# PolyChord/PolyChordLite

Measured on AMD Instinct MI355X. Metric: likelihood evals/sec, 20D Gaussian nlive=2000, higher is better.
Workload: dtype f64; 1 GPU; configs[1]: 20-D Gaussian, nlive=2000, num_repeats=40, one full run per step; batch_chains=1000, parallelism=repeat-sharded x1, mode=one run at a time per GPU; R runs in step: roofline.in_step

## Files before the change

### polychordlite_amd/csrc/pc_sample.hip

```cpp
#include "pc_state.h"
#ifndef __HIPCC_RTC__
#include <cstdlib>
#endif

template <int DPL>
struct LaneDims {
    double lo[DPL], span[DPL];
    double mean[DPL];
    bool on[DPL];
};

__device__ __forceinline__ double pc_box_theta(double lo, double span, double cube) { return lo + span * cube; }
#define PC_PT_SORTED (1u << 16)
#define PC_PT_PERMUTED (1u << 17)
#define PC_PT_ADAPTIVE (1u << 18)
#define PC_PT_LAYER (1u << 19)
template <int DPL>
struct LaneTable {
    int type[DPL], pos[DPL], len[DPL], hyp[DPL];
    int cnt[DPL], lay[DPL];
    double p0[DPL], p1[DPL], p2[DPL];
    unsigned mask;
};
template <int DPL, bool AD>
// ... 1011 lines not shown
    if (off > 0) {
        for (int e = tid; e < Dg * D; e += NT) G[e] = 0.0;
        __syncthreads();
    }
    for (uint32_t call = (e0 >> 1) + tid; call <= ((e1 - 1) >> 1); call += NT) {
        double ua, ub;
        if (S.seq_mode) pc_uniform2(S.k0, S.k1, PC_DOM_SEQ, 0u, 0u, call, ua, ub);
        else pc_uniform2(S.k0, S.k1, PC_DOM_NHAT, batch, (uint32_t)chain, call, ua, ub);
        const uint32_t ia = 2 * call, ib = 2 * call + 1;
        if (ia >= e0 && ia < e1) { const uint32_t x = ia - e0; G[off == 0 ? x : (x / Dg) * D + off + x % Dg] = pc_inv_normal_cdf(ua); }
        if (ib >= e0 && ib < e1) { const uint32_t x = ib - e0; G[off == 0 ? x : (x / Dg) * D + off + x % Dg] = pc_inv_normal_cdf(ub); }
    }
    __syncthreads();
#ifdef NHATS_DBG
    ncyc[2] = clock64();
#endif
#pragma unroll
    for (int d = 0; d < DMAX; ++d) v[d] = (active && d < D) ? G[(size_t)i * D + d] : 0.0;
#define PC_DOT4(RES, A, B) { double p0_ = 0.0, p1_ = 0.0, p2_ = 0.0, p3_ = 0.0; \
        _Pragma("unroll") for (int d = 0; d < DMAX; d += 4) { \
            p0_ += (A)[d] * (B)[d]; p1_ += (A)[d + 1] * (B)[d + 1]; p2_ += (A)[d + 2] * (B)[d + 2]; p3_ += (A)[d + 3] * (B)[d + 3]; } \
        RES = (p0_ + p1_) + (p2_ + p3_); }
    {
        double n2;
        PC_DOT4(n2, v, v)
        const double inrm = 1.0 / sqrt(n2);
#pragma unroll
        for (int d = 0; d < DMAX; ++d) v[d] = v[d] * inrm;
    }
#ifdef NHATS_DBG
    ncyc[3] = clock64();
#endif
    double *Qb = Q;
    const int QS = DMAX;
    if (i == 0) {
#pragma unroll
        for (int d = 0; d < DMAX; ++d) Qb[d] = v[d];
    }
    __syncthreads();
#define PC_GS_STEP(QV) { \
        double qq, dv; \
        PC_DOT4(qq, QV, QV) \
        PC_DOT4(dv, QV, v) \
        if (i == j) { \
            const double inrm = 1.0 / sqrt(qq); \
            _Pragma("unroll") for (int d = 0; d < DMAX; ++d) v[d] = v[d] * inrm; \
        } else if (active && i > j) { \
            const double cproj = dv / qq; \
            _Pragma("unroll") for (int d = 0; d < DMAX; ++d) v[d] = v[d] - cproj * (QV)[d]; \
            if (i == j + 1) { \
                double *qn = Qb + (size_t)((j + 1) & 1) * QS; \
                _Pragma("unroll") for (int d = 0; d < DMAX; ++d) qn[d] = v[d]; \
            } \
        } }
    for (int j = 0; j < Dg; ++j) {
        const double *q = Qb + (size_t)(j & 1) * QS;
        if constexpr (DMAX <= 32) {
            double qv[DMAX];
#pragma unroll
            for (int d = 0; d < DMAX; ++d) qv[d] = q[d];
            PC_GS_STEP(qv)
        } else {
            PC_GS_STEP(q)
        }
        __syncthreads();
    }
#undef PC_GS_STEP
    if constexpr (PART == 1) {
        if (active) {
#pragma unroll
            for (int d = 0; d < DMAX; ++d) if (d < D) raw[d] = v[d];
        }
        return;
    }
    }
#ifdef NHATS_DBG
    ncyc[4] = clock64();
#endif
    const int col = col0 + basis * Dg + i;
    const bool wanted = basis * Dg + i < nrg;
    if constexpr (DMAX <= 32) {
        const double *Lg = S.chol + (size_t)sh[0] * D * D;
        for (int e = tid; e < D * D; e += NT) G[e] = Lg[e];
        __syncthreads();
        if (active && wanted) {
            double t[DMAX];
#pragma unroll
            for (int a = 0; a < DMAX; ++a) t[a] = 0.0;
#pragma unroll
            for (int b = 0; b < DMAX; ++b)
#pragma unroll
                for (int a = b; a < DMAX; ++a) t[a] += G[(size_t)a * D + b] * v[b];
#pragma unroll
            for (int a = 0; a < DMAX; ++a) if (a >= D) t[a] = 0.0;
            double n2;
            PC_DOT4(n2, t, t)
            const double w = sqrt(n2), iw = 1.0 / w;
            double *out = S.nhat + ((size_t)chain * nr + col) * D;
#pragma unroll
            for (int d = 0; d < DMAX; ++d) if (d < D) out[d] = t[d] * iw;
            S.nhat_w[(size_t)chain * nr + col] = w * 3.0;
        }
    } else {
        const int DS = D + 1, TR = 12;
        double *Lt = G + (size_t)D * DS;
        __syncthreads();
        if (active) {
#pragma unroll
            for (int d = 0; d < DMAX; ++d) if (d < D) G[(size_t)i * DS + d] = v[d];
        }
        const double *Lc = S.chol + (size_t)sh[0] * D * D;
        double *mine = G + (size_t)i * DS;
        for (int a_hi = D - 1; a_hi >= 0; a_hi -= TR) {
            const int a_lo = max(0, a_hi - TR + 1), nrow = a_hi - a_lo + 1;
            __syncthreads();
            for (int e = tid; e < nrow * D; e += NT) Lt[e] = Lc[(size_t)a_lo * D + e];
            __syncthreads();
            if (active && wanted) {
                for (int a = a_hi; a >= a_lo; --a) {
                    const double *Lr = Lt + (size_t)(a - a_lo) * D;
                    double t0 = 0.0, t1 = 0.0, t2 = 0.0, t3 = 0.0;
                    int bb = 0;
                    for (; bb + 3 <= a; bb += 4) {
                        t0 += Lr[bb] * mine[bb]; t1 += Lr[bb + 1] * mine[bb + 1]; t2 += Lr[bb + 2] * mine[bb + 2]; t3 += Lr[bb + 3] * mine[bb + 3];
                    }
                    for (; bb <= a; ++bb) t0 += Lr[bb] * mine[bb];
                    mine[a] = (t0 + t1) + (t2 + t3);
                }
            }
        }
        if (active && wanted) {
            double n0 = 0.0, n1 = 0.0;
            int d = 0;
            for (; d + 1 < D; d += 2) { n0 += mine[d] * mine[d]; n1 += mine[d + 1] * mine[d + 1]; }
            if (d < D) n0 += mine[d] * mine[d];
            const double w = sqrt(n0 + n1);
            Q[i] = 1.0 / w;
            S.nhat_w[(size_t)chain * nr + col] = w * 3.0;
        }
        __syncthreads();
        for (int r = 0; r < Dg && basis * Dg + r < nrg; ++r) {
            double *out = S.nhat + ((size_t)chain * nr + col0 + basis * Dg + r) * D;
            const double iw = Q[r];
            for (int d = tid; d < D; d += NT) out[d] = G[(size_t)r * DS + d] * iw;
        }
    }
#ifdef NHATS_DBG
    ncyc[5] = clock64();
    if (tid == 0 && blockIdx.x == 0 && blockIdx.y == 0) for (int x = 0; x < 5; ++x) S.ctl->dbg[x] += ncyc[x + 1] - ncyc[x];
#endif
#undef PC_DOT4
}

template <int DMAX>
__global__ __launch_bounds__(64) void k_nhats_w(PcState S, unsigned batch, int nbases)
{
    extern __shared__ __attribute__((aligned(16))) char smem[];
    const int D = S.D, DD = D * D, nb = S.nb_total, nr = S.nr, per = 64 / D, NC = (DD + 1) / 2;
    const int tid = threadIdx.x, sub = tid / D, i = tid - sub * D;
    const int g0 = blockIdx.x * per, g = g0 + sub;
    const int nbw = nbases - g0 < per ? nbases - g0 : per;
    const bool active = sub < per && g < nbases;
    double *G = (double *)smem;
    double *Qw = G + (size_t)per * DD;
    int *qA = (int *)(Qw + (size_t)per * 2 * DMAX);
    if (nr <= 64) {
        for (int s = 0; s < nbw; ++s) {
            const int chain = (g0 + s) / nb;
            if (g0 + s != chain * nb) continue;
            const int dk = pc_deck_keyed(S, batch, chain, tid, nr);
            int *rec = pc_deck_record(S, chain);
            rec[2 + tid] = dk;
            const unsigned long long tg = pc_deck_tag(S, batch, chain, nr);
            if (tid == 0) { rec[0] = (int)(unsigned)tg; rec[1] = (int)(unsigned)(tg >> 32); }
        }
    }
    int qn = 0;
    auto put = [&](bool want, double u, int dst) {
        bool t = false;
        double x = 0.0;
        if (want) x = pc_inv_normal_central(u, t);
        if (want) G[dst] = t ? u : x;
        const unsigned long long m = __ballot(want && t);
        if (want && t) qA[qn + __popcll(m & ((1ull << tid) - 1ull))] = dst;
        qn += __popcll(m);
    };
    for (int t0 = 0; t0 < nbw * NC; t0 += 64) {
        const int t = t0 + tid;
        const bool in = t < nbw * NC;
        const int s = in ? t / NC : 0, m = in ? t - s * NC : 0;
        const int chain = (g0 + s) / nb, basis = (g0 + s) - chain * nb;
        const uint32_t e0 = (uint32_t)pc_sel(S.g_e0, 0) + (uint32_t)basis * DD, e1 = e0 + (uint32_t)DD;
        const uint32_t call = (e0 >> 1) + (uint32_t)m;
        double ua = 0.5, ub = 0.5;
        if (in) pc_uniform2(S.k0, S.k1, PC_DOM_NHAT, batch, (uint32_t)chain, call, ua, ub);
        const uint32_t ia = 2 * call, ib = ia + 1;
        put(in && ia >= e0 && ia < e1, ua, s * DD + (int)(ia - e0));
        put(in && ib >= e0 && ib < e1, ub, s * DD + (int)(ib - e0));
    }
    __syncthreads();
    for (int k = tid; k < qn; k += 64) { const int at = qA[k]; G[at] = pc_inv_normal_tail(G[at]); }
    __syncthreads();
    double v[DMAX];
    const double *mine = G + (size_t)(active ? sub : 0) * DD + (size_t)i * D;
#pragma unroll
    for (int d = 0; d < DMAX; ++d) v[d] = (active && d < D) ? mine[d] : 0.0;
    double *Q = Qw + (size_t)(sub < per ? sub : 0) * 2 * DMAX;
    {
#pragma clang fp contract(off)
        PC_GS_PACKED(DMAX, v, Q, D, i, active)
    }
    if (active) {
        double *raw = S.nhat_raw + ((size_t)g * D + i) * D;
#pragma unroll
        for (int d = 0; d < DMAX; ++d) if (d < D) raw[d] = v[d];
    }
}

#define PC_BIG_NT 256
#define PC_BIG_P 16
__global__ __launch_bounds__(PC_BIG_NT) void k_nhats_big(PcState S, unsigned batch)
{
    __shared__ int sh[2];
    __shared__ double iwv[PC_BIG_NT];
    __shared__ double Pq[PC_BIG_P * PC_BIG_NT];
    __shared__ double pqq[PC_BIG_P];
    const int D = S.D, nr = S.nr, tid = threadIdx.x, chain = blockIdx.y, i = tid;
    int grade, basis;
    pc_grade_of_basis(S, blockIdx.x, grade, basis);
    const int off = pc_sel(S.g_off, grade), Dg = D - off, nrg = pc_sel(S.g_nr, grade), col0 = pc_sel(S.g_col0, grade);
    if (tid == 0) {
        int sel, slot;
        select_seed(S, batch, chain, sel, slot);
        sh[0] = sel; sh[1] = slot;
        if (blockIdx.x == 0) {
            S.ch_cluster[chain] = sel; S.ch_seed_slot[chain] = slot;
            S.ch_contour[chain] = S.logLp[sel];
            S.ch_epoch[chain] = S.ctl->admin_epoch;
            if (chain == 0) { S.ctl->i_nursery = gridDim.y; S.ctl->batch_id = batch; }
        }
    }
    double *V = S.nhat_raw + ((size_t)chain * gridDim.x + blockIdx.x) * D * PC_BIG_NT;
    const int nvec = min(Dg, nrg - basis * Dg);
    const bool active = i < nvec;
    const uint32_t eoff = S.seq_mode ? (uint32_t)S.ctl->seq + 2u : 0u;
    const uint32_t e0 = eoff + (uint32_t)pc_sel(S.g_e0, grade) + (uint32_t)basis * Dg * Dg, e1 = e0 + (uint32_t)Dg * Dg;
    for (int e = tid; e < off * PC_BIG_NT; e += PC_BIG_NT) V[e] = 0.0;
    for (uint32_t call = (e0 >> 1) + tid; call <= ((e1 - 1) >> 1); call += PC_BIG_NT) {
        double ua, ub;
        if (S.seq_mode) pc_uniform2(S.k0, S.k1, PC_DOM_SEQ, 0u, 0u, call, ua, ub);
        else pc_uniform2(S.k0, S.k1, PC_DOM_NHAT, batch, (uint32_t)chain, call, ua, ub);
        const uint32_t ia = 2 * call, ib = 2 * call + 1;
        if (ia >= e0 && ia < e1) { const uint32_t x = ia - e0; V[(size_t)(off + x % Dg) * PC_BIG_NT + x / Dg] = pc_inv_normal_cdf(ua); }
        if (ib >= e0 && ib < e1) { const uint32_t x = ib - e0; V[(size_t)(off + x % Dg) * PC_BIG_NT + x / Dg] = pc_inv_normal_cdf(ub); }
    }
    __syncthreads();
    double *mine = V + i;
    auto dot_own = [&](const double *q) {
        double p0 = 0.0, p1 = 0.0, p2 = 0.0, p3 = 0.0;
        int d = off;
        for (; d + 3 < D; d += 4) {
            p0 += q[(size_t)d * PC_BIG_NT] * mine[(size_t)d * PC_BIG_NT]; p1 += q[(size_t)(d + 1) * PC_BIG_NT] * mine[(size_t)(d + 1) * PC_BIG_NT];
            p2 += q[(size_t)(d + 2) * PC_BIG_NT] * mine[(size_t)(d + 2) * PC_BIG_NT]; p3 += q[(size_t)(d + 3) * PC_BIG_NT] * mine[(size_t)(d + 3) * PC_BIG_NT];
        }
        for (; d < D; ++d) p0 += q[(size_t)d * PC_BIG_NT] * mine[(size_t)d * PC_BIG_NT];
        return (p0 + p1) + (p2 + p3);
    };
    auto norm2 = [&](const double *q) {
        double p0 = 0.0, p1 = 0.0, p2 = 0.0, p3 = 0.0;
        int d = off;
        for (; d + 3 < D; d += 4) {
            const double a = q[(size_t)d * PC_BIG_NT], b = q[(size_t)(d + 1) * PC_BIG_NT], c = q[(size_t)(d + 2) * PC_BIG_NT], e = q[(size_t)(d + 3) * PC_BIG_NT];
            p0 += a * a; p1 += b * b; p2 += c * c; p3 += e * e;
        }
        for (; d < D; ++d) { const double a = q[(size_t)d * PC_BIG_NT]; p0 += a * a; }
        return (p0 + p1) + (p2 + p3);
    };
    if (active) {
        const double inrm = 1.0 / sqrt(dot_own(mine));
        for (int d = off; d < D; ++d) mine[(size_t)d * PC_BIG_NT] *= inrm;
    }
    __syncthreads();
    {
        const int wv = tid >> 6, lane = tid & 63;
        for (int j0 = 0; j0 < nvec; j0 += PC_BIG_P) {
            const int np = min(PC_BIG_P, nvec - j0);
            for (int e = tid; e < np * D; e += PC_BIG_NT) {
                const int pp = e % np, d = e / np;
                Pq[pp * PC_BIG_NT + d] = V[(size_t)d * PC_BIG_NT + j0 + pp];
            }
            for (int e = np * PC_BIG_NT + tid; e < PC_BIG_P * PC_BIG_NT; e += PC_BIG_NT) Pq[e] = 0.0;
            __syncthreads();
            for (int pp = 0; pp + 1 < np; ++pp) {
                const double *qp = Pq + pp * PC_BIG_NT;
                for (int q = pp + 1 + wv; q < np; q += 4) {
                    double *vq = Pq + q * PC_BIG_NT;
                    double dq = 0.0, dd = 0.0;
                    for (int d = off + lane; d < D; d += 64) { const double a = qp[d], b2 = vq[d]; dq += a * b2; dd += a * a; }
                    dq = wave_sum<4>(dq); dd = wave_sum<4>(dd);
                    const double c = dq / dd;
                    for (int d = off + lane; d < D; d += 64) vq[d] -= c * qp[d];
                }
                __syncthreads();
            }
            for (int pp = wv; pp < np; pp += 4) {
                const double *qp = Pq + pp * PC_BIG_NT;
                double dd = 0.0;
                for (int d = off + lane; d < D; d += 64) dd += qp[d] * qp[d];
                dd = wave_sum<4>(dd);
                if (lane == 0) pqq[pp] = dd;
            }
            for (int e = tid; e < np * D; e += PC_BIG_NT) {
                const int pp = e % np, d = e / np;
                V[(size_t)d * PC_BIG_NT + j0 + pp] = Pq[pp * PC_BIG_NT + d];
            }
            __syncthreads();
            if (active && i >= j0 + np) {
                double c[PC_BIG_P];
#pragma unroll
                for (int pp = 0; pp < PC_BIG_P; ++pp) c[pp] = 0.0;
                for (int d = off; d < D; ++d) {
                    const double x = mine[(size_t)d * PC_BIG_NT];
#pragma unroll
                    for (int pp = 0; pp < PC_BIG_P; ++pp) c[pp] += x * Pq[pp * PC_BIG_NT + d];
                }
#pragma unroll
                for (int pp = 0; pp < PC_BIG_P; ++pp) c[pp] = pp < np ? c[pp] / pqq[pp] : 0.0;
                for (int d = off; d < D; ++d) {
                    double x = mine[(size_t)d * PC_BIG_NT];
#pragma unroll
                    for (int pp = 0; pp < PC_BIG_P; ++pp) x -= c[pp] * Pq[pp * PC_BIG_NT + d];
                    mine[(size_t)d * PC_BIG_NT] = x;
                }
            }
            __syncthreads();
        }
    }
    if (active) {
        const double inrm = 1.0 / sqrt(dot_own(mine));
        for (int d = off; d < D; ++d) mine[(size_t)d * PC_BIG_NT] *= inrm;
    }
    {
        const double *Lc = S.chol + (size_t)sh[0] * D * D;
        for (int a_hi = D - 1; a_hi >= 0; a_hi -= PC_BIG_P) {
            const int a_lo = max(0, a_hi - PC_BIG_P + 1), nrow = a_hi - a_lo + 1;
            __syncthreads();
            for (int e = tid; e < PC_BIG_P * PC_BIG_NT; e += PC_BIG_NT) {
                const int r = e / PC_BIG_NT, b2 = e % PC_BIG_NT;
                Pq[e] = (r < nrow && b2 <= a_hi) ? Lc[(size_t)(a_lo + r) * D + b2] : 0.0;
            }
            __syncthreads();
            if (active) {
                double acc[PC_BIG_P];
#pragma unroll
                for (int r = 0; r < PC_BIG_P; ++r) acc[r] = 0.0;
                for (int b2 = 0; b2 <= a_hi; ++b2) {
                    const double x = mine[(size_t)b2 * PC_BIG_NT];
#pragma unroll
                    for (int r = 0; r < PC_BIG_P; ++r) acc[r] += Pq[r * PC_BIG_NT + b2] * x;
                }
#pragma unroll
                for (int r = 0; r < PC_BIG_P; ++r) if (r < nrow) mine[(size_t)(a_lo + r) * PC_BIG_NT] = acc[r];
            }
        }
    }
    if (active) {
        double sn = 0.0, cn = 0.0;
        for (int d = 0; d < D; ++d) {
#pragma clang fp contract(off)
// ... 550 lines not shown
        if (kind == PC_LIKE_SOURCE) {
            lA = oa ? C.S.logzero : like_eval<DPL, NROWS, KIND>(C.S, thA, C.ld, C.lane, C.ybuf);
            lB = ob ? C.S.logzero : like_eval<DPL, NROWS, KIND>(C.S, thB, C.ld, C.lane, C.ybuf);
            if (!oa && lA > C.S.logzero) C.nlike++;
            if (!ob && lB > C.S.logzero) C.nlike++;
            return;
        }
#endif
        lA = like_eval<DPL, NROWS, KIND>(C.S, thA, C.ld, C.lane, C.ybuf);
        lB = like_eval<DPL, NROWS, KIND>(C.S, thB, C.ld, C.lane, C.ybuf);
        if (oa) lA = C.S.logzero; else if (lA > C.S.logzero) C.nlike++;
        if (ob) lB = C.S.logzero; else if (lB > C.S.logzero) C.nlike++;
        return;
    }
    bool outA = false, outB = false;
    double sA = 0.0, sB = 0.0, s2A = 0.0, s2B = 0.0;
#pragma unroll
    for (int k = 0; k < DPL; ++k) {
        const double cA = x0[k] + tA * nh[k], cB = x0[k] + tB * nh[k];
        if (C.ld.on[k]) { outA |= (cA < 0.0) | (cA > 1.0); outB |= (cB < 0.0) | (cB > 1.0); }
        const double thA = C.ld.lo[k] + C.ld.span[k] * cA, thB = C.ld.lo[k] + C.ld.span[k] * cB;
        if (C.ld.on[k]) {
            if (kind == PC_LIKE_RASTRIGIN) {
                sA += 8.515435146961291 + thA * thA - 10.0 * cos(PC_TWO_PI * thA);
                sB += 8.515435146961291 + thB * thB - 10.0 * cos(PC_TWO_PI * thB);
            } else {
                const int dim = C.lane + 64 * k;
                const double m1 = dim < 2 ? -0.5 : 0.0, m2 = dim < 2 ? 0.5 : 0.0;
                const double a1 = (thA - m1) * L.inv_sigma, a2 = (thA - m2) * L.inv_sigma;
                const double b1 = (thB - m1) * L.inv_sigma, b2 = (thB - m2) * L.inv_sigma;
                sA += a1 * a1; s2A += a2 * a2; sB += b1 * b1; s2B += b2 * b2;
            }
        }
    }
    const bool oa = __ballot(outA) != 0ull, ob = __ballot(outB) != 0ull;
    sA = wsum<DPL, NROWS>(sA); sB = wsum<DPL, NROWS>(sB);
    if (kind == PC_LIKE_RASTRIGIN) { lA = -sA; lB = -sB; }
    else {
        s2A = wsum<DPL, NROWS>(s2A); s2B = wsum<DPL, NROWS>(s2B);
        lA = pc_logaddexp(L.norm - sA / 2.0, L.norm - s2A / 2.0) - 0.6931471805599453;
        lB = pc_logaddexp(L.norm - sB / 2.0, L.norm - s2B / 2.0) - 0.6931471805599453;
    }
    if (oa) lA = C.S.logzero; else if (lA > C.S.logzero) C.nlike++;
    if (ob) lB = C.S.logzero; else if (lB > C.S.logzero) C.nlike++;
}

#ifndef PC_STEP_SPEC
#define PC_STEP_SPEC 1
#endif
constexpr int pc_step_spec = PC_STEP_SPEC;
#ifdef PC_SLICE_WAVES
#define PC_SLICE_ATTR __attribute__((amdgpu_waves_per_eu(PC_SLICE_WAVES, PC_SLICE_WAVES)))
#else
#define PC_SLICE_ATTR
#endif
template <int DPL, int NROWS, bool SPECIAL, int WPB = 1, int FW = 0, int LEAN = 0, int PT = 0>
__global__ PC_SLICE_ATTR __launch_bounds__(64 * WPB * ((FW > 0 && (LEAN == 1 || LEAN == 3 || LEAN == 5) && WPB == 4) ? 2 : 1)) void k_slice(PcState S, unsigned batch, int phi_lds, int mat_lds)
{
#include "pc_slice_body.inc"
}

template <int DPL, int NROWS, bool SPECIAL, int WPB = 1, int FW = 0, int LEAN = 0, int PT = 0>
__global__ PC_SLICE_ATTR __launch_bounds__(64 * WPB) void k_slice_many(const PcManyRec *__restrict__ R, int phi_lds, int mat_lds)
{
    const PcState S = R[blockIdx.y].S;
    const unsigned batch = (unsigned)R[blockIdx.y].ia[PC_REC_I_BATCH];
#include "pc_slice_body.inc"
}

#ifndef __HIPCC_RTC__
#include "pc_launch.h"
#include <cstdio>
extern "C" int pc_rtc_wanted(const PcState *S) { return S->like.kind == PC_LIKE_SOURCE || (S->ablate & PC_ABL_RTC_BUILTINS) != 0; }
template <class... A> static int pc_rtc_go(const PcState *S, const char *expr, dim3 g, dim3 b, size_t sh, hipStream_t st, A... a)
{
    void *args[] = { (void *)&a... };
    return pc_rtc_launch(S, expr, g, b, sh, st, args);
}
#define PC_LAUNCH(K, G, B, SH, ST, ...) do { if (pc_rtc_wanted(S)) { if (pc_rtc_go(S, #K, G, B, SH, ST, __VA_ARGS__)) return 1; } \
                                             else hipLaunchKernelGGL(K, G, B, SH, ST, __VA_ARGS__); } while (0)
static size_t pc_terms_lds(const PcState *S, const PcSourceForm &f, int phi_lds)
{
    if (f.nterms <= 0) return 0;
    return sizeof(double) * ((size_t)S->D + (phi_lds ? (size_t)S->nr * (size_t)f.nsums : 0)) + pc_front_lds(f);
}
static PcSourceForm pc_state_form(const PcState *S)
{
    PcSourceForm f{};
    if (S->like.kind == PC_LIKE_SOURCE) (void)pc_rtc_source_form(S->src_id, &f);
    return f;
}
static int pc_dpl(int D) { return D <= 64 ? 1 : (D <= 128 ? 2 : (D <= 256 ? 4 : 0)); }
extern "C" int pc_launch_generate_live(const PcState *S, int attempt0, int n, double *rows, double *rows_logL,
                                       hipStream_t st)
{
    const size_t sh = sizeof(double) * S->D + pc_front_lds(pc_state_form(S));
    const bool table = S->prior.kind >= 2;
    switch (pc_dpl(S->D) + (table ? 8 : 0)) {
    case 1: PC_LAUNCH((k_generate_live<1>), dim3(n), dim3(64), sh, st, *S, attempt0, rows, rows_logL); return 0;
    case 2: PC_LAUNCH((k_generate_live<2>), dim3(n), dim3(64), sh, st, *S, attempt0, rows, rows_logL); return 0;
    case 4: PC_LAUNCH((k_generate_live<4>), dim3(n), dim3(64), sh, st, *S, attempt0, rows, rows_logL); return 0;
    case 9: PC_LAUNCH((k_generate_live<1, 1>), dim3(n), dim3(64), sh, st, *S, attempt0, rows, rows_logL); return 0;
    case 10: PC_LAUNCH((k_generate_live<2, 1>), dim3(n), dim3(64), sh, st, *S, attempt0, rows, rows_logL); return 0;
    case 12: PC_LAUNCH((k_generate_live<4, 1>), dim3(n), dim3(64), sh, st, *S, attempt0, rows, rows_logL); return 0;
    }
    return 1;
}

extern "C" int pc_nhats_splittable(const PcState *S)
{
    const char *e = std::getenv("PC_NHATS_QUAD_MIN");
    if (S->D > 64 && S->D <= 128) return S->ngrade <= 1 && !S->seq_mode && S->nhat_raw != nullptr;
    if (S->D > 24 && S->D <= 64) return S->ngrade <= 1 && !S->seq_mode && S->nhat_raw != nullptr && (!e || std::atoi(e) <= 25);
    return S->D <= 24 && S->D < (e ? std::atoi(e) : 25) && !S->seq_mode && S->nhat_raw != nullptr;
}
static size_t pc_nhats_q_lds(int HV) { return sizeof(double) * (size_t)(2 + HV) * 4 * (HV + 2); }
static size_t pc_nhats_q32_lds(int D) { const int NR = ((D + 15) / 16) * 16; return sizeof(double) * (2 * 4 * 34 + (size_t)(NR + (NR <= 112 ? 32 : 16)) * 129); }
static size_t pc_nhats_w_lds(int D, int DMAX) { return (size_t)(64 / D) * (sizeof(double) * ((size_t)D * D + 2 * DMAX) + sizeof(int) * (size_t)D * D); }
extern "C" int pc_launch_nhats_part(const PcState *S, unsigned batch, int nchains, int part, hipStream_t st, int packed)
{
    if (!pc_nhats_splittable(S)) return 1;
    const int D = S->D;
    dim3 grid(S->nb_total, nchains);
    if (D > 64) {
        if (part == 1) {
            static const bool panel_off = std::getenv("PC_BASIS_PANEL_OFF") != nullptr;
            const int nt1 = (D + 15) / 16;
            if (panel_off) hipLaunchKernelGGL((k_nhats_q<32, 1>), grid, dim3(512), sizeof(double) * 2 * 4 * 34, st, *S, batch);
            else if (nt1 <= 5) hipLaunchKernelGGL((k_basis<5>), grid, dim3(512), 0, st, *S, batch);
            else if (nt1 == 6) hipLaunchKernelGGL((k_basis<6>), grid, dim3(512), 0, st, *S, batch);
            else if (nt1 == 7) hipLaunchKernelGGL((k_basis<7>), grid, dim3(512), 0, st, *S, batch);
            else hipLaunchKernelGGL((k_basis<8>), grid, dim3(512), 0, st, *S, batch);
        }
        else {
            dim3 g2(S->nb_total * 2, nchains);
            const int nt = (D + 15) / 16;
            if (nt <= 5) hipLaunchKernelGGL((k_whiten<5>), g2, dim3(256), 0, st, *S, batch);
            else if (nt == 6) hipLaunchKernelGGL((k_whiten<6>), g2, dim3(256), 0, st, *S, batch);
            else if (nt == 7) hipLaunchKernelGGL((k_whiten<7>), g2, dim3(256), 0, st, *S, batch);
            else hipLaunchKernelGGL((k_whiten<8>), g2, dim3(256), 0, st, *S, batch);
        }
        return 0;
    }
    if (D > 24) {
        if (D <= 32) { if (part == 1) hipLaunchKernelGGL((k_nhats_q<8, 1>), grid, dim3(128), pc_nhats_q_lds(8), st, *S, batch); else hipLaunchKernelGGL((k_nhats_q<8, 2>), grid, dim3(128), pc_nhats_q_lds(8), st, *S, batch); }
        else { if (part == 1) hipLaunchKernelGGL((k_nhats_q<16, 1>), grid, dim3(256), pc_nhats_q_lds(16), st, *S, batch); else hipLaunchKernelGGL((k_nhats_q<16, 2>), grid, dim3(256), pc_nhats_q_lds(16), st, *S, batch); }
        return 0;
    }
    const size_t sh = sizeof(double) * ((size_t)(D + 8) * (D + 8) + 2 * 128) + 16;
    if (part == 1 && packed == PC_PART1_PACKED && pc_launch_bases_t(S, batch, nchains, st) == 0) return 0;
    if (part == 1 && packed == PC_PART1_WAVE && S->ngrade <= 1) {
        const int nbases = nchains * S->nb_total, per = 64 / D;
        const dim3 gw((nbases + per - 1) / per);
        if (D <= 8) hipLaunchKernelGGL((k_nhats_w<8>), gw, dim3(64), pc_nhats_w_lds(D, 8), st, *S, batch, nbases);
        else if (D <= 16) hipLaunchKernelGGL((k_nhats_w<16>), gw, dim3(64), pc_nhats_w_lds(D, 16), st, *S, batch, nbases);
        else hipLaunchKernelGGL((k_nhats_w<24>), gw, dim3(64), pc_nhats_w_lds(D, 24), st, *S, batch, nbases);
        return 0;
    }
    if (part == 1) {
        if (D <= 8) hipLaunchKernelGGL((k_nhats<8, 64, 1>), grid, dim3(64), sh, st, *S, batch);
        else if (D <= 16) hipLaunchKernelGGL((k_nhats<16, 64, 1>), grid, dim3(64), sh, st, *S, batch);
        else hipLaunchKernelGGL((k_nhats<24, 64, 1>), grid, dim3(64), sh, st, *S, batch);
    } else {
        if (D <= 8) hipLaunchKernelGGL((k_nhats<8, 64, 2>), grid, dim3(64), sh, st, *S, batch);
        else if (D <= 16) hipLaunchKernelGGL((k_nhats<16, 64, 2>), grid, dim3(64), sh, st, *S, batch);
        else hipLaunchKernelGGL((k_nhats<24, 64, 2>), grid, dim3(64), sh, st, *S, batch);
    }
    return 0;
}

extern "C" int pc_launch_nhats(const PcState *S, unsigned batch, int nchains, hipStream_t st)
{
    const int D = S->D, nb = S->nb_total;
    dim3 grid(nb, nchains);
    static int quad_min = -1;
    if (quad_min < 0) { const char *e = std::getenv("PC_NHATS_QUAD_MIN"); quad_min = e ? std::atoi(e) : 25; }
    if (D >= quad_min) {
        if (D <= 32) hipLaunchKernelGGL((k_nhats_q<8>), grid, dim3(128), pc_nhats_q_lds(8), st, *S, batch);
        else if (D <= 64) hipLaunchKernelGGL((k_nhats_q<16>), grid, dim3(256), pc_nhats_q_lds(16), st, *S, batch);
        else if (D <= 128) {
            const size_t shq = pc_nhats_q32_lds(D);
            pc_need_dyn_lds((const void *)k_nhats_q<32>, shq);
            hipLaunchKernelGGL((k_nhats_q<32>), grid, dim3(512), shq, st, *S, batch);
        }
        else if (D <= 256 && S->nhat_raw) hipLaunchKernelGGL(k_nhats_big, grid, dim3(PC_BIG_NT), 0, st, *S, batch);
        else return 1;
        return 0;
    }
    const size_t sh = sizeof(double) * ((size_t)(D + 8) * (D + 8) + 2 * 128) + 16;
    if (D <= 8) hipLaunchKernelGGL((k_nhats<8, 64>), grid, dim3(64), sh, st, *S, batch);
    else if (D <= 16) hipLaunchKernelGGL((k_nhats<16, 64>), grid, dim3(64), sh, st, *S, batch);
    else if (D <= 24) hipLaunchKernelGGL((k_nhats<24, 64>), grid, dim3(64), sh, st, *S, batch);
    else if (D <= 32) hipLaunchKernelGGL((k_nhats<32, 64>), grid, dim3(64), sh, st, *S, batch);
    else if (D <= 64) hipLaunchKernelGGL((k_nhats<64, 64>), grid, dim3(64), sh, st, *S, batch);
    else return 1;
    return 0;
}

extern "C" int pc_launch_nhats_many(const PcState *S, const PcManyRec *dR, int R, int nchains, hipStream_t st)
{
    const int D = S->D, nb = S->nb_total;
    if (D < 25 || D > 64 || S->seq_mode || std::getenv("PC_NHATS_QUAD_MIN")) return 1;
    dim3 grid(nb, nchains, R);
    if (D <= 32) hipLaunchKernelGGL((k_nhats_q_many<8>), grid, dim3(128), pc_nhats_q_lds(8), st, dR);
    else hipLaunchKernelGGL((k_nhats_q_many<16>), grid, dim3(256), pc_nhats_q_lds(16), st, dR);
    return 0;
}

extern "C" int pc_slice_fusable(const PcState *S)
{
    static const bool off = std::getenv("PC_SLICE_FUSED_OFF") != nullptr;
    return !off && S->D <= 24 && pc_nhats_splittable(S) && S->ngrade <= 1 && S->like.kind != PC_LIKE_CORR_GAUSSIAN && S->nr <= 1024;
}

static int pc_table_pt(const PcState *S) { return S->prior.kind == 2 && ((unsigned)S->src_pad & PC_PT_ADAPTIVE) ? 2 : 1; }
struct PcSlicePlan {
    bool ok, many;
    int dpl, nrows; bool special; int wpb, fw, lean, pt;
    dim3 grid, block; size_t lds;
    int phi_lds, mat_lds;
};

static PcSlicePlan pc_slice_plan(const PcState *S, int nchains, int fused, int R)
{
    static const bool lean_off = std::getenv("PC_SLICE_LEAN_OFF") != nullptr, helper_off = std::getenv("PC_SLICE_HELPER_OFF") != nullptr,
                      wpb_off = std::getenv("PC_SLICE_WPB_OFF") != nullptr;
    PcSlicePlan p{};
    const int D = S->D, nr = S->nr;
    const bool table = S->prior.kind >= 2;
    const bool special = S->ngrade > 1 || S->seq_mode;
    const bool corr = S->like.kind == PC_LIKE_CORR_GAUSSIAN;
    if (D > 256 || (fused && !pc_slice_fusable(S))) return p;
    if (R && (table || (!fused && (corr || special || D > 64)))) return p;
    p.many = R > 0;
    p.dpl = pc_dpl(D);
    p.nrows = D <= 16 ? 1 : ((D <= 32 || fused) ? 2 : 4);
    p.special = special; p.wpb = 1; p.pt = table ? pc_table_pt(S) : 0;
    p.fw = !fused ? 0 : (D <= 8 ? 8 : (D <= 16 ? 16 : 24));
    p.grid = R ? dim3(nchains, R) : dim3(nchains); p.block = dim3(64);
    const PcSourceForm f = pc_state_form(S);
    p.phi_lds = pc_slice_phi_lds(S, f);
    const size_t tb = sizeof(double) * (size_t)nr * (D + 1);
    size_t sh = sizeof(double) * ((size_t)D + nr) + 16 + (p.phi_lds ? tb : 0);
    if (fused) sh += sizeof(double) * ((size_t)p.fw * D + (size_t)nr * (D + 2));
    if (!R) sh += pc_terms_lds(S, f, p.phi_lds);
    if (fused && sh > 150 * 1024) return p;
    int leanf = 0;
    if (!lean_off && !special && !table)
        leanf = S->like.kind == PC_LIKE_RASTRIGIN ? 3 : (S->like.kind == PC_LIKE_TWIN_GAUSSIAN ? 4 : ((S->like.kind == PC_LIKE_GAUSSIAN && (S->ablate & PC_ABL_FUNCTOR) && !R) ? 5 : 0));
    if (fused) {
        const bool lean = !R && !lean_off && !table && S->like.kind == PC_LIKE_GAUSSIAN && !(S->ablate & PC_ABL_FUNCTOR) && p.phi_lds && nr <= 64 && !special;
        p.lean = leanf ? leanf : (lean ? 1 : 0);
        const size_t pw4 = ((size_t)D + nr + (p.phi_lds ? (size_t)nr * (D + 1) : 0) + (size_t)p.fw * D + (size_t)nr * (D + 2) + (size_t)((nr + 3) / 4) * 128 + (size_t)nr + 1) & ~(size_t)1;
        const size_t sh4 = 4 * sizeof(double) * pw4 + 16;
        if (!R && (p.lean == 1 || p.lean == 3 || p.lean == 5) && !helper_off && !(S->ablate & PC_ABL_NO_HELPER) && nr <= 64 && (nchains & 3) == 0 && sh4 <= 150 * 1024) {
            p.wpb = 4; p.grid = dim3(nchains / 4); p.block = dim3(512); sh = sh4;
        }
    } else {
        const size_t mb = sizeof(double) * (size_t)D * D;
        p.mat_lds = (!table && corr && S->nhat_Ms == nullptr && sh + mb <= 150 * 1024) ? 1 : 0;
        if (p.mat_lds && D > 64 && D <= 128 && nchains % 4 == 0 && !special && !wpb_off && 4 * sh + mb <= 150 * 1024) {
            p.wpb = 4; p.grid = dim3(nchains / 4); p.block = dim3(256); sh = 4 * sh + mb;
        } else {
            if (p.mat_lds) sh += mb;
            if (!lean_off && !table && corr && S->nhat_Ms != nullptr && !(S->ablate & PC_ABL_FUNCTOR) && S->nDer == 0 && nr > 64 && D > 64 && D <= 128 && !special) p.lean = 2;
            else if (D <= 64) p.lean = leanf;
        }
    }
    p.lds = sh; p.ok = true;
    return p;
}

#define PC_SLICE_ADAPT_VARIANTS(X) \
    X(1, 1, false, 1, 0, 0, 2) X(1, 1, true, 1, 0, 0, 2) X(1, 2, false, 1, 0, 0, 2) X(1, 2, true, 1, 0, 0, 2) X(1, 4, false, 1, 0, 0, 2) X(1, 4, true, 1, 0, 0, 2) X(2, 4, false, 1, 0, 0, 2) X(2, 4, true, 1, 0, 0, 2) X(4, 4, false, 1, 0, 0, 2) X(4, 4, true, 1, 0, 0, 2) X(1, 1, false, 1, 8, 0, 2) X(1, 1, false, 1, 16, 0, 2) X(1, 2, false, 1, 24, 0, 2)
#define PC_SLICE_STEP_ADAPT_VARIANTS(X) \
    X(1, 1, false, 1, 0, 0, 2) X(1, 2, false, 1, 0, 0, 2) X(1, 4, false, 1, 0, 0, 2) X(1, 1, false, 1, 8, 0, 2) X(1, 1, false, 1, 16, 0, 2) X(1, 2, false, 1, 24, 0, 2)

#define PC_SLICE_VARIANTS(X) \
     \
    X(1, 1, false, 1, 0, 0, 0) X(1, 1, true, 1, 0, 0, 0) X(1, 1, false, 1, 0, 0, 1) X(1, 1, true, 1, 0, 0, 1) X(1, 1, false, 1, 0, 3, 0) X(1, 1, false, 1, 0, 4, 0) X(1, 1, false, 1, 0, 5, 0) \
    X(1, 2, false, 1, 0, 0, 0) X(1, 2, true, 1, 0, 0, 0) X(1, 2, false, 1, 0, 0, 1) X(1, 2, true, 1, 0, 0, 1) X(1, 2, false, 1, 0, 3, 0) X(1, 2, false, 1, 0, 4, 0) X(1, 2, false, 1, 0, 5, 0) \
    X(1, 4, false, 1, 0, 0, 0) X(1, 4, true, 1, 0, 0, 0) X(1, 4, false, 1, 0, 0, 1) X(1, 4, true, 1, 0, 0, 1) X(1, 4, false, 1, 0, 3, 0) X(1, 4, false, 1, 0, 4, 0) X(1, 4, false, 1, 0, 5, 0) \
    X(2, 4, false, 1, 0, 0, 0) X(2, 4, true, 1, 0, 0, 0) X(2, 4, false, 1, 0, 0, 1) X(2, 4, true, 1, 0, 0, 1) \
    X(4, 4, false, 1, 0, 0, 0) X(4, 4, true, 1, 0, 0, 0) X(4, 4, false, 1, 0, 0, 1) X(4, 4, true, 1, 0, 0, 1) \
     \
    X(2, 4, false, 4, 0, 0, 0) X(2, 4, false, 1, 0, 2, 0) \
     \
     \
    X(1, 1, false, 1, 8, 0, 0) X(1, 1, false, 1, 8, 0, 1) X(1, 1, false, 1, 8, 1, 0) X(1, 1, false, 4, 8, 1, 0) X(1, 1, false, 1, 8, 3, 0) X(1, 1, false, 4, 8, 3, 0) X(1, 1, false, 1, 8, 4, 0) X(1, 1, false, 4, 8, 4, 0) X(1, 1, false, 1, 8, 5, 0) X(1, 1, false, 4, 8, 5, 0) \
    X(1, 1, false, 1, 16, 0, 0) X(1, 1, false, 1, 16, 0, 1) X(1, 1, false, 1, 16, 1, 0) X(1, 1, false, 4, 16, 1, 0) X(1, 1, false, 1, 16, 3, 0) X(1, 1, false, 4, 16, 3, 0) X(1, 1, false, 1, 16, 4, 0) X(1, 1, false, 4, 16, 4, 0) X(1, 1, false, 1, 16, 5, 0) X(1, 1, false, 4, 16, 5, 0) \
    X(1, 2, false, 1, 24, 0, 0) X(1, 2, false, 1, 24, 0, 1) X(1, 2, false, 1, 24, 1, 0) X(1, 2, false, 4, 24, 1, 0) X(1, 2, false, 1, 24, 3, 0) X(1, 2, false, 4, 24, 3, 0) X(1, 2, false, 1, 24, 4, 0) X(1, 2, false, 4, 24, 4, 0) X(1, 2, false, 1, 24, 5, 0) X(1, 2, false, 4, 24, 5, 0)
#define PC_SLICE_MANY_VARIANTS(X) \
    X(1, 1, false, 1, 0, 0) X(1, 1, false, 1, 0, 3) X(1, 1, false, 1, 0, 4) X(1, 2, false, 1, 0, 0) X(1, 2, false, 1, 0, 3) X(1, 2, false, 1, 0, 4) X(1, 4, false, 1, 0, 0) X(1, 4, false, 1, 0, 3) X(1, 4, false, 1, 0, 4) \
    X(1, 1, false, 1, 8, 0) X(1, 1, false, 1, 8, 3) X(1, 1, false, 1, 8, 4) X(1, 1, false, 1, 16, 0) X(1, 1, false, 1, 16, 3) X(1, 1, false, 1, 16, 4) X(1, 2, false, 1, 24, 0) X(1, 2, false, 1, 24, 3) X(1, 2, false, 1, 24, 4)

static int pc_slice_launch(const PcState *S, const PcSlicePlan &p, const PcManyRec *dR, unsigned batch, hipStream_t st)
{
    if (!p.ok) return 1;
#define PC_ROW(DPL, NROWS, SPECIAL, WPB, FW, LEAN, PT) \
    if (!p.many && p.dpl == DPL && p.nrows == NROWS && p.special == SPECIAL && p.wpb == WPB && p.fw == FW && p.lean == LEAN && p.pt == PT) { \
        if (p.lds > 48 * 1024) pc_need_dyn_lds((const void *)k_slice<DPL, NROWS, SPECIAL, WPB, FW, LEAN, PT>, p.lds); \
        PC_LAUNCH((k_slice<DPL, NROWS, SPECIAL, WPB, FW, LEAN, PT>), p.grid, p.block, p.lds, st, *S, batch, p.phi_lds, p.mat_lds); \
        return 0; }
    PC_SLICE_VARIANTS(PC_ROW)
    PC_SLICE_ADAPT_VARIANTS(PC_ROW)
#undef PC_ROW
#define PC_ROW(DPL, NROWS, SPECIAL, WPB, FW, LEAN) \
    if (p.many && p.dpl == DPL && p.nrows == NROWS && p.special == SPECIAL && p.wpb == WPB && p.fw == FW && p.lean == LEAN && p.pt == 0) { \
        if (p.lds > 48 * 1024) pc_need_dyn_lds((const void *)k_slice_many<DPL, NROWS, SPECIAL, WPB, FW, LEAN>, p.lds); \
// ... 121 lines not shown
```

### polychordlite_amd/csrc/pc_state.h

```cpp
#pragma once
#include "pc_dev.h"

enum { PC_ST_RUNNING = 0, PC_ST_DONE = 1, PC_ST_UPDATE = 2, PC_ST_ERROR = 4 };
enum { PC_ERR_NONE = 0, PC_ERR_PHANTOM_CAP = 1, PC_ERR_DEAD_CAP = 2, PC_ERR_CLUSTER_CAP = 3, PC_ERR_NOSLOT = 4 };

enum { PC_ABL_FUNCTOR = 1 << 0, PC_ABL_NO_POOL = 1 << 1, PC_ABL_NO_DEFER = 1 << 2, PC_ABL_NO_FUSED_UPDATE = 1 << 3, PC_ABL_PAIR_SCANS = 1 << 4,
       PC_ABL_CONSUME_GENERAL = 1 << 5, PC_ABL_SLICE_LANE = 1 << 6, PC_ABL_BASES_PACKED = 1 << 7, PC_ABL_CL_END_AT_DEATH = 1 << 8,
       PC_ABL_KILLOFF_GENERAL = 1 << 9, PC_ABL_CONSUME_CL_SERIAL = 1 << 10, PC_ABL_RETIRED_11 = 1 << 11, PC_ABL_RETIRED_12 = 1 << 12,
       PC_ABL_NO_HELPER = 1 << 13, PC_ABL_QC_BY_CHAIN = 1 << 14, PC_ABL_RTC_BUILTINS = 1 << 15, PC_ABL_UPDATE_CHAIN = 1 << 16, PC_ABL_FLAG_LAUNCH = 1 << 17,
       PC_ABL_ACCEPT_SERIAL = 1 << 18, PC_ABL_BASES_WAVE = 1 << 19, PC_ABL_TRACE_CHOL = 1 << 30 };

#define PC_MASK_WORDS 16

struct PcCtl {
    int status;
    int error;
    int i_nursery;
    int admin_epoch;
    int failures;
    int ncluster;
    int ncluster_dead;
    int ndead;
    int nphantom;
    int seg_hi, seg_lo;
    int cluster_deleted;
    unsigned batch_id;
    unsigned next_cluster_uid;
    long long nlike;
    long long niter;
    long long nlike_device;
    long long nlike_failed;
    double logZ, logZ2;
    double logX_last_update;
    double live_logZ;
    unsigned long long seq;
    long long dbg[8];
    long long gen_cyc[4];
    long long nn_walks, nn_fallbacks;
    int upd_pending, upd_marks;
    int upd_tmark;
    int upd_T, upd_ts;
    int upd_nph0;
    int upd_keep_thr;
    int fin_ndead0;
    double upd_thr;
    int chol_suspect;
    int fin_n0;
    long long wave_cyc[4];
};

#define PC_MAX_GRADE 8
#define PC_NN_K 8
#define PC_NN_NONE (-2147483647 - 1)
#define PC_CUID_NONE 0xFFFFFFFEu

struct alignas(16) PcPlanHead {
    int dead_idx;
    int dead_src;
    int ph_base;
    unsigned dead_cuid;
    unsigned ph_cuid;
    int ph_count;
    double logw;
    double postX, postZ;
    double postXs;
    double contour;
};
struct alignas(16) PcPlan : PcPlanHead {
    unsigned long long ph_mask[PC_MASK_WORDS];
};
static_assert(sizeof(PcPlanHead) == 64 && sizeof(PcPlan) == 64 + 8 * PC_MASK_WORDS, "plan record layout");

struct PcState {
    int D, nDer, nT, nr, N, Ncap, B, maxc, Pcap, Dcap;
    int b0, l0, p0, d0;
    uint32_t k0, k1;
    double logzero, log_prec, log_cf;
    int use_prec, max_ndead, nfail;
    int n_nlives; const double *dyn_loglikes; const int *dyn_nlives;
    PcLike like; PcPrior prior;
    double *live;
    double *live_logL;
    int *live_cluster;
    int *live_pos;
    double *live_entry;
    int *cl_list;
    int *cl_n;
    double *logZp, *logXp, *logZXp, *logZp2, *logZpXp, *logLp, *XpXq ;
    int *imin_slot;
    double *lse_ref, *lse_sum;
    double *death_thr;
    unsigned *cl_uid;
    double *chol, *cov;
    double *logZp_dead, *logZp2_dead;
    unsigned *cl_uid_dead;
    int maxc_dead;
    double *phantom;
    double *ph_logL;
    unsigned *ph_cuid;
    unsigned long long *ph_uid;
    double *dead;
    double *dead_logw;
    double *dead_postX, *dead_postZ;
    unsigned *dead_cuid;
    double *dead_entry;
    double *babies;
    double *baby_logL;
    double *baby_logL_T;
    int *ch_cluster, *ch_epoch, *ch_nlike, *ch_seed_slot;
    double *ch_contour;
    double *nhat;
    double *nhat_w;
    double *nhat_raw;
    double *nhat_Ms;
    double *ch_My;
    PcPlan *plan;
    int *sort_slot;
    unsigned long long *sort_key;
    int *slot_src;
    int *slot_dead;
    int *slot_step;
    int defer_update;
    int pool, pool_base, pool_rows;
    int ngrade, nb_total; unsigned n_dev;
    int g_off[PC_MAX_GRADE], g_nr[PC_MAX_GRADE], g_nb[PC_MAX_GRADE], g_col0[PC_MAX_GRADE], g_e0[PC_MAX_GRADE];
    int *ch_nlike_g;
    const double *logn;
    int *nn_list;
    int *nn_slot_owner;
    int *nn_chain_slot;
    double *nn_pts;
    int *nn_code;
    int nn_valid;
    int ablate;
    int seq_mode;
    int epoch_discard;
    int seed_override;
    PcCtl *ctl;
    PcCtl *ctl_host; unsigned notify_seq;
    int src_id, src_pad;
    const double *src_data; long long src_ndata;
};

struct PcManyRec { PcState S; void *p[10]; int ia[6]; int pad[2]; };
enum { PC_REC_I_BATCH = 0, PC_REC_I_BASES_SEQ = 3 };
enum { PC_REC_KEEP = 0, PC_REC_BLK = 1, PC_REC_TOTAL = 2, PC_REC_PH2 = 3, PC_REC_PHL2 = 4, PC_REC_PHC2 = 5, PC_REC_PHU2 = 6, PC_REC_PART = 7, PC_REC_SHIFT = 8 };
enum { PC_REC_I_ROWS = 1, PC_REC_I_BLOCKS = 2 };
enum { PC_REC_I_NLEFT = 1 };
enum { PC_REC_DESC = 0, PC_REC_SM = 1, PC_REC_KNN = 2, PC_REC_LAB = 3, PC_REC_OUT = 4, PC_REC_DIMS = 5 };
enum { PC_REC_I_ND = 1, PC_REC_I_NMAX = 2, PC_REC_I_ND_SUB = 3 };
enum { PC_REC_G_DESC = 0, PC_REC_G_SM = 1, PC_REC_G_POOL = 2, PC_REC_G_KNN = 3, PC_REC_G_LAB = 4, PC_REC_G_OUT = 5 };
enum { PC_REC_I_NB = 1, PC_REC_I_MMAX = 2 };
enum { PC_REC_T_CS = 0, PC_REC_T_X0 = 1, PC_REC_T_DECK = 2, PC_REC_T_PROP = 3, PC_REC_T_LOGL = 4, PC_REC_T_THETA = 5, PC_REC_T_PHI = 6, PC_REC_T_RANK = 7 };
enum { PC_REC_I_FIRST = 1 };

struct PcParkRun { const int *need; const double *prop; int *rank; int nchains, stride; };
#define PC_PARK_MAX_RUNS 64

#ifdef __HIPCC__
template <class T, class B> __device__ __forceinline__ T *pc_as_global(T *p, const B * )
{
    typedef __attribute__((address_space(1))) char gchar;
    return (T *)(gchar *)(uintptr_t)p;
// ... 97 lines not shown
```

Before: 1.402 billion likelihood evals/s.

## Run wave-packed basis kernel with four waves per block, offloading deck generation

The wave-packed random-basis kernel now launches with four wavefronts per block. All four waves share the uniform-draw and inverse-normal work, with an LDS atomic counter collecting tail entries. After that, wave 0 does the Gram-Schmidt while waves 1-3 generate the per-chain deck records in parallel. Wave 0 stages its output in LDS and writes it back as a contiguous coalesced copy. This spreads the RNG and deck cost across more lanes, at the price of an extra barrier, LDS atomics and three waves that sit idle during orthogonalisation. The old single-wave path remains behind a new ablation flag, and optional clock64 instrumentation is added.

```diff
diff --git a/polychordlite_amd/csrc/pc_sample.hip b/polychordlite_amd/csrc/pc_sample.hip
--- a/polychordlite_amd/csrc/pc_sample.hip
+++ b/polychordlite_amd/csrc/pc_sample.hip
@@ -1187,40 +1187,68 @@
 #undef PC_DOT4
 }
 
-template <int DMAX>
-__global__ __launch_bounds__(64) void k_nhats_w(PcState S, unsigned batch, int nbases)
+template <int DMAX, int NW>
+__global__ __launch_bounds__(64 * NW) void k_nhats_w(PcState S, unsigned batch, int nbases)
 {
     extern __shared__ __attribute__((aligned(16))) char smem[];
     const int D = S.D, DD = D * D, nb = S.nb_total, nr = S.nr, per = 64 / D, NC = (DD + 1) / 2;
-    const int tid = threadIdx.x, sub = tid / D, i = tid - sub * D;
+    const int tid = threadIdx.x, lane = NW == 1 ? tid : (tid & 63), wv = NW == 1 ? 0 : __builtin_amdgcn_readfirstlane(tid >> 6);
+    const int sub = lane / D, i = lane - sub * D;
     const int g0 = blockIdx.x * per, g = g0 + sub;
     const int nbw = nbases - g0 < per ? nbases - g0 : per;
     const bool active = sub < per && g < nbases;
     double *G = (double *)smem;
     double *Qw = G + (size_t)per * DD;
     int *qA = (int *)(Qw + (size_t)per * 2 * DMAX);
-    if (nr <= 64) {
+#ifdef NHATS_W_DBG
+    long long wcy[8];
+    wcy[0] = wcy[1] = clock64();
+#define NHATS_W_MARK(k) wcy[k] = clock64();
+#else
+#define NHATS_W_MARK(k)
+#endif
+    auto decks = [&]() {
+        if (nr > 64) return;
+        int ns = 0;
         for (int s = 0; s < nbw; ++s) {
             const int chain = (g0 + s) / nb;
             if (g0 + s != chain * nb) continue;
-            const int dk = pc_deck_keyed(S, batch, chain, tid, nr);
-            int *rec = pc_deck_record(S, chain);
-            rec[2 + tid] = dk;
-            const unsigned long long tg = pc_deck_tag(S, batch, chain, nr);
-            if (tid == 0) { rec[0] = (int)(unsigned)tg; rec[1] = (int)(unsigned)(tg >> 32); }
-        }
-    }
+            if (NW == 1 || wv == 1 + ns % (NW > 1 ? NW - 1 : 1)) {
+                const int dk = pc_deck_keyed(S, batch, chain, lane, nr);
+                int *rec = pc_deck_record(S, chain);
+                rec[2 + lane] = dk;
+                const unsigned long long tg = pc_deck_tag(S, batch, chain, nr);
+                if (lane == 0) { rec[0] = (int)(unsigned)tg; rec[1] = (int)(unsigned)(tg >> 32); }
+            }
+            ++ns;
+        }
+    };
+    if constexpr (NW == 1) { decks(); NHATS_W_MARK(1) }
     int qn = 0;
+    int *qcnt = nullptr;
+    if constexpr (NW > 1) {
+        __shared__ int qcnt_s;
+        qcnt = &qcnt_s;
+        if (tid == 0) qcnt_s = 0;
+        __syncthreads();
+    }
     auto put = [&](bool want, double u, int dst) {
         bool t = false;
         double x = 0.0;
         if (want) x = pc_inv_normal_central(u, t);
         if (want) G[dst] = t ? u : x;
         const unsigned long long m = __ballot(want && t);
-        if (want && t) qA[qn + __popcll(m & ((1ull << tid) - 1ull))] = dst;
-        qn += __popcll(m);
+        if constexpr (NW == 1) {
+            if (want && t) qA[qn + __popcll(m & ((1ull << tid) - 1ull))] = dst;
+            qn += __popcll(m);
+        } else if (m) {
+            int at = 0;
+            if (lane == 0) at = atomicAdd(qcnt, __popcll(m));
+            at = __builtin_amdgcn_readfirstlane(at);
+            if (want && t) qA[at + __popcll(m & ((1ull << lane) - 1ull))] = dst;
+        }
     };
-    for (int t0 = 0; t0 < nbw * NC; t0 += 64) {
+    for (int t0 = 0; t0 < nbw * NC; t0 += 64 * NW) {
         const int t = t0 + tid;
         const bool in = t < nbw * NC;
         const int s = in ? t / NC : 0, m = in ? t - s * NC : 0;
@@ -1234,22 +1262,63 @@
         put(in && ib >= e0 && ib < e1, ub, s * DD + (int)(ib - e0));
     }
     __syncthreads();
-    for (int k = tid; k < qn; k += 64) { const int at = qA[k]; G[at] = pc_inv_normal_tail(G[at]); }
+    NHATS_W_MARK(2)
+    if constexpr (NW > 1) qn = *qcnt;
+    for (int k = tid; k < qn; k += 64 * NW) { const int at = qA[k]; G[at] = pc_inv_normal_tail(G[at]); }
     __syncthreads();
+    NHATS_W_MARK(3)
+    if constexpr (NW > 1) {
+        if (wv != 0) {
+            decks();
+#ifdef NHATS_W_DBG
+            if (wv == 1 && lane == 0 && (NHATS_W_DBG == 2 || blockIdx.x == 0)) atomicAdd((unsigned long long *)&S.ctl->dbg[0], (unsigned long long)(clock64() - wcy[3]));
+#endif
+            return;
+        }
+    }
     double v[DMAX];
     const double *mine = G + (size_t)(active ? sub : 0) * DD + (size_t)i * D;
 #pragma unroll
     for (int d = 0; d < DMAX; ++d) v[d] = (active && d < D) ? mine[d] : 0.0;
     double *Q = Qw + (size_t)(sub < per ? sub : 0) * 2 * DMAX;
+#ifdef NHATS_W_DBG
+    {
+        double sv = 0.0;
+#pragma unroll
+        for (int d = 0; d < DMAX; ++d) sv += v[d];
+        asm volatile("" :: "v"(sv));
+    }
+#endif
+    NHATS_W_MARK(4)
     {
 #pragma clang fp contract(off)
         PC_GS_PACKED(DMAX, v, Q, D, i, active)
     }
-    if (active) {
+    NHATS_W_MARK(5)
+    if constexpr (NW > 1) {
+        double *row = G + (size_t)(active ? sub : 0) * DD + (size_t)i * D;
+        if (active) {
+#pragma unroll
+            for (int d = 0; d < DMAX; ++d) if (d < D) row[d] = v[d];
+        }
+        __syncthreads();
+        double *raw0 = S.nhat_raw + (size_t)g0 * DD;
+        for (int e = lane; e < nbw * DD; e += 64) raw0[e] = G[e];
+    } else if (active) {
         double *raw = S.nhat_raw + ((size_t)g * D + i) * D;
 #pragma unroll
         for (int d = 0; d < DMAX; ++d) if (d < D) raw[d] = v[d];
     }
+#ifdef NHATS_W_DBG
+    asm volatile("s_waitcnt vmcnt(0)" ::: "memory");
+    NHATS_W_MARK(6)
+    if (lane == 0 && (NHATS_W_DBG == 2 || blockIdx.x == 0)) {
+        for (int x = (NW == 1 ? 0 : 1); x < 6; ++x) atomicAdd((unsigned long long *)&S.ctl->dbg[x], (unsigned long long)(wcy[x + 1] - wcy[x]));
+        atomicAdd((unsigned long long *)&S.ctl->dbg[6], (unsigned long long)(wcy[6] - wcy[0]));
+        atomicAdd((unsigned long long *)&S.ctl->dbg[7], 1ull);
+    }
+#endif
+#undef NHATS_W_MARK
 }
 
 #define PC_BIG_NT 256
@@ -2106,9 +2175,15 @@
     if (part == 1 && packed == PC_PART1_WAVE && S->ngrade <= 1) {
         const int nbases = nchains * S->nb_total, per = 64 / D;
         const dim3 gw((nbases + per - 1) / per);
-        if (D <= 8) hipLaunchKernelGGL((k_nhats_w<8>), gw, dim3(64), pc_nhats_w_lds(D, 8), st, *S, batch, nbases);
-        else if (D <= 16) hipLaunchKernelGGL((k_nhats_w<16>), gw, dim3(64), pc_nhats_w_lds(D, 16), st, *S, batch, nbases);
-        else hipLaunchKernelGGL((k_nhats_w<24>), gw, dim3(64), pc_nhats_w_lds(D, 24), st, *S, batch, nbases);
+        if (S->ablate & PC_ABL_BASES_WAVE1) {
+            if (D <= 8) hipLaunchKernelGGL((k_nhats_w<8, 1>), gw, dim3(64), pc_nhats_w_lds(D, 8), st, *S, batch, nbases);
+            else if (D <= 16) hipLaunchKernelGGL((k_nhats_w<16, 1>), gw, dim3(64), pc_nhats_w_lds(D, 16), st, *S, batch, nbases);
+            else hipLaunchKernelGGL((k_nhats_w<24, 1>), gw, dim3(64), pc_nhats_w_lds(D, 24), st, *S, batch, nbases);
+            return 0;
+        }
+        if (D <= 8) hipLaunchKernelGGL((k_nhats_w<8, 4>), gw, dim3(256), pc_nhats_w_lds(D, 8), st, *S, batch, nbases);
+        else if (D <= 16) hipLaunchKernelGGL((k_nhats_w<16, 4>), gw, dim3(256), pc_nhats_w_lds(D, 16), st, *S, batch, nbases);
+        else hipLaunchKernelGGL((k_nhats_w<24, 4>), gw, dim3(256), pc_nhats_w_lds(D, 24), st, *S, batch, nbases);
         return 0;
     }
     if (part == 1) {
diff --git a/polychordlite_amd/csrc/pc_state.h b/polychordlite_amd/csrc/pc_state.h
--- a/polychordlite_amd/csrc/pc_state.h
+++ b/polychordlite_amd/csrc/pc_state.h
@@ -8,7 +8,7 @@
        PC_ABL_CONSUME_GENERAL = 1 << 5, PC_ABL_SLICE_LANE = 1 << 6, PC_ABL_BASES_PACKED = 1 << 7, PC_ABL_CL_END_AT_DEATH = 1 << 8,
        PC_ABL_KILLOFF_GENERAL = 1 << 9, PC_ABL_CONSUME_CL_SERIAL = 1 << 10, PC_ABL_RETIRED_11 = 1 << 11, PC_ABL_RETIRED_12 = 1 << 12,
        PC_ABL_NO_HELPER = 1 << 13, PC_ABL_QC_BY_CHAIN = 1 << 14, PC_ABL_RTC_BUILTINS = 1 << 15, PC_ABL_UPDATE_CHAIN = 1 << 16, PC_ABL_FLAG_LAUNCH = 1 << 17,
-       PC_ABL_ACCEPT_SERIAL = 1 << 18, PC_ABL_BASES_WAVE = 1 << 19, PC_ABL_TRACE_CHOL = 1 << 30 };
+       PC_ABL_ACCEPT_SERIAL = 1 << 18, PC_ABL_BASES_WAVE = 1 << 19, PC_ABL_BASES_WAVE1 = 1 << 20, PC_ABL_TRACE_CHOL = 1 << 30 };
 
 #define PC_MASK_WORDS 16
 
```

After: 1.435 billion likelihood evals/s, median of 6. 2.3% higher.
